# danieleschmidt/spin-torque-rl-gym

Measured on AMD Instinct MI355X. Metric: env_steps_per_sec, higher is better.
Workload: dtype f64

## Files before the change

### spin-torque-rl-gym_amd/csrc/stg_kernels.hpp

```cpp
#pragma once
#include "../../include/spintorque_hip.h"
#include "stg_launch_plan.hpp"
#include "stg_physics.hpp"

#include <hip/hip_runtime.h>

#include <type_traits>

using namespace stg;

struct alignas(16) EnvRec {
    double m[3];
    double tgt[3];
    double etot;
    uint32_t stepw;
    uint32_t rng;
};
static_assert(sizeof(EnvRec) == 64, "state record size");
constexpr uint32_t STG_DONE_BIT = 0x80000000u;

struct StateView {
    EnvRec* rec;
};

// ... 507 lines not shown
        } else {
            const int64_t p = IDS ? o : i;
            parse_action<AT>(act[p], act[N + p], a.c.max_current, a.c.max_duration, J, T);
        }
        if (MULTI) {
            const int c = (int)a.cls[i];
            row = s_tab + (c < a.ncls ? c : 0) * C_COUNT;
            k = load_llgs(row);
        }
        const RngKey rk{a.c.seed, (uint64_t)(a.env_id0 + i), rng};
        e_skip = a.c.skip_done && done;
        llgs_lane_begin<THERMAL, false, AXIS_Z>(L, out_m, m, J, T, k, row[C_BETA], row[C_BETAP], a.c.rtol, a.c.atol, a.c.max_step, rk,
                                                norec, noek, ns, !e_skip);
        has_env = true;
    };
    auto finish = [&]() {
        const SolveOut so = llgs_lane_finish<false>(L, out_m, norec, noek, ns);
        V3 m = L.m0, tgt = e_tgt;
        double etot = e_etot;
        int32_t step = e_step;
        uint32_t rng = e_rng;
        bool done = e_skip;
        env_step_tail(a, IDS ? o : i, 0, true, true, !e_skip, row, (uint64_t)(a.env_id0 + i), m, tgt, etot, step, rng, done, J, T, so, c_steps, c_sub, c_noop);
        store_state(a.s, i, m, tgt, etot, step, rng, done);
        has_env = false;
        L.active = false;
    };

    take(w * 64 + lane, true);
    const int64_t n_rest = nblk_q > nw ? nblk_q - nw : 0;
    static_assert(REFILL_STRIPES == 64, "one lane per stripe when a wavefront looks for a stripe that still has entries");
    int stripe = (int)(w % REFILL_STRIPES);
    bool queue_open = true;
    int64_t loc_q = 0, loc_end = 0;
    int loc_stripe = 0, full_streak = 0;
    bool more = n_rest > 0;
    const int check = a.refill_check > 0 ? a.refill_check : 1;
    for (;;) {
        LlgsMasks M = llgs_masks_open(L);
        for (int c = 0; c < check; ++c) {
            llgs_lane_gate<false>(L, M, (int32_t)a.c.max_attempts);
            if (M.active == 0ull) break;
            V3 z2{0.0, 0.0, 0.0}, z3{0.0, 0.0, 0.0};
            llgs_lane_attempt<THERMAL, false, AXIS_Z, false>(L, M, out_m, k, tb, a.c.rtol, a.c.atol, a.c.max_step, norec, noek, ns, z2, z3);
        }
        llgs_masks_close(L, M);
        const bool fin = has_env && !L.active;
        if (__ballot(fin) != 0ull || (more && __ballot(!has_env) != 0ull)) {
            if (fin) finish();
            const unsigned long long takers = __ballot(!has_env);
            if (more && takers != 0ull) {
                const int n_take = (int)__builtin_popcountll(takers), first = (int)__builtin_ctzll(takers);
                const int rank = (int)__builtin_popcountll(takers & ((1ull << lane) - 1ull));
                const int64_t avail = loc_end - loc_q;
                const int need_new = n_take > avail ? (int)(n_take - avail) : 0;
                int64_t new_q = 0;
                const int new_stripe = stripe;
                if (need_new > 0 && queue_open) {
                    const int reserve = (takers == ~0ull && full_streak >= 1) ? 4 * 64 : need_new;
                    unsigned long long base = 0;
                    if (lane == first) base = atomicAdd(a.refill_cursor + stripe * REFILL_CURSOR_STRIDE, (unsigned long long)reserve);
                    base = (unsigned long long)__shfl((long long)base, first);
                    new_q = (int64_t)base;
                    const int64_t stripe_end = ((n_rest - stripe + REFILL_STRIPES - 1) / REFILL_STRIPES) * 64;
                    int64_t new_end = new_q + reserve;
                    if (new_end >= stripe_end) {
                        new_end = stripe_end;
                        const int64_t end_l = ((n_rest - lane + REFILL_STRIPES - 1) / REFILL_STRIPES) * 64;
                        const unsigned long long cur_l = __hip_atomic_load(a.refill_cursor + lane * REFILL_CURSOR_STRIDE, __ATOMIC_RELAXED, __HIP_MEMORY_SCOPE_AGENT);
                        unsigned long long open_s = __ballot((int64_t)cur_l < end_l);
                        open_s &= ~(1ull << stripe);
                        if (open_s == 0ull) queue_open = false;
                        else {
                            const unsigned long long after = stripe == 63 ? 0ull : (open_s >> (stripe + 1)) << (stripe + 1);
                            stripe = (int)__builtin_ctzll(after != 0ull ? after : open_s);
                        }
                    }
                    const bool from_old = rank < avail;
                    const int64_t q = from_old ? loc_q + rank : new_q + (rank - avail);
                    const int st = from_old ? loc_stripe : new_stripe;
                    const int64_t r = (q >> 6) * REFILL_STRIPES + st;
                    take((nw + r) * 64 + (q & 63), !has_env && r < n_rest && (from_old || q < new_end));
                    loc_q = new_q + need_new < new_end ? new_q + need_new : new_end;
                    loc_end = new_end;
                    loc_stripe = new_stripe;
                } else {
                    const int64_t q = loc_q + rank;
                    const int64_t r = (q >> 6) * REFILL_STRIPES + loc_stripe;
                    take((nw + r) * 64 + (q & 63), !has_env && q < loc_end && r < n_rest);
                    loc_q = loc_q + n_take < loc_end ? loc_q + n_take : loc_end;
                }
                more = queue_open || loc_q < loc_end;
                full_streak = takers == ~0ull ? full_streak + 1 : 0;
            }
        }
        if (__ballot(has_env) == 0ull && !more) break;
    }
}

template <int SOLVER, bool THERMAL, int MULTI, bool AXIS_Z, bool DEVPHYS, typename AT, bool PC, int WGW, bool IDS>
#ifndef STG_STEP_ATTR
#define STG_STEP_ATTR
#endif
__global__ void __launch_bounds__(PC ? 2 * WGW * 64 : WGW * 64, (SOLVER != STG_SOLVER_RK45 && !THERMAL && !DEVPHYS && AXIS_Z && MULTI != 2 && !(MULTI && WGW == 1)) ? 4 : 1) STG_STEP_ATTR
stg_step_kernel(const StepArgs a) {
#pragma clang fp contract(off)
    static_assert(!PC || THERMAL, "wave specialisation only exists for the thermal kernels");
    extern __shared__ double s_tab[];
    constexpr bool FIELD = SOLVER == STG_SOLVER_RK45;
    using NT = typename std::conditional<FIELD, double, float>::type;
    constexpr bool BARRIER = SOLVER != STG_SOLVER_RK4;
    constexpr int DEPTH = BARRIER ? 2 : 4;
    constexpr int RING = DEPTH * (FIELD ? SHARED_CHUNK_RK45 : SHARED_CHUNK_FIXED) * 64;
    static_assert(!PC || WGW == 1, "the wave-specialised form is one integrating + one producing wavefront");
    __shared__ NT s_norm[PC ? RING : 1];
    __shared__ int s_hs[2], s_go[2 * WGW];
    __shared__ unsigned long long s_cnt[(PC ? 2 : 1) * WGW * 3];
    __shared__ uint32_t s_rng[PC ? WGW * 64 : 1];
    const int lane = (int)(threadIdx.x & 63u);
    const int wave = __builtin_amdgcn_readfirstlane((int)(threadIdx.x >> 6));
    bool paired = PC;
    int64_t hyb_slot = 0;
    if (PC && a.hybrid) hyb_slot = stg_hybrid_block(blockIdx.x, wave, (uint32_t)(a.hybrid - 1), (a.N + TILE_ENVS - 1) / TILE_ENVS, paired);
    const bool producer = PC && paired && wave >= WGW;
    const int cw = producer ? (2 * WGW - 1 - wave) : (wave < WGW ? wave : wave - WGW);
    record_placement(a.placement, wave, lane, producer);
    const int64_t lane_slot = ((PC && a.hybrid) ? hyb_slot
                                                : stg_slot_block<WGW>(blockIdx.x, (uint32_t)((a.N + WGW * 64 - 1) / (WGW * 64)), a.perm != nullptr, cw, PC,
                                                                      (uint32_t)a.snake_rounds) * 64) + lane;
    const bool in_list = lane_slot < a.N;
    const int64_t o = in_list ? (a.perm ? (int64_t)a.perm[lane_slot] : lane_slot) : 0;
    const uint32_t id = (IDS && in_list) ? a.ids[o] : 0u;
    const bool bad = IDS && in_list && (int64_t)id >= a.n_state;
    if (bad && !producer) write_bad_id(a, o);
    const bool live = in_list && !bad;
    const int64_t i = IDS ? (live ? (int64_t)id : 0) : o;
    constexpr int ENV_LAYOUT = SOLVER == STG_SOLVER_RK45 ? ENV_LAYOUT_LLGS : (DEVPHYS ? ENV_LAYOUT_DEV : ENV_LAYOUT_CORE);
    double own_row[MULTI == 2 ? C_COUNT : 1];
    const double* row;
    if constexpr (MULTI == 2) {
        stg_device_params p;
        load_env_params<ENV_LAYOUT>(a.ep, i, p);
        derive_row(p, a.ep.gamma, a.ep.temperature, own_row);
        row = own_row;
    } else {
        row = class_row<MULTI != 0>(a.ctab, a.cls, a.ncls, i, live, s_tab, a.ep, ENV_LAYOUT);
    }
    if (!PC && !live) return;
    if (PC && !paired && !live) return;
    const int64_t N = a.N;
    const uint64_t env_id = (uint64_t)(a.env_id0 + i);

    if (producer) {
        constexpr int n_first = SOLVER == STG_SOLVER_RK45 ? 6 : SHARED_CHUNK_FIXED;
        static_assert(3 * SHARED_SUBS3 == SHARED_CHUNK_FIXED, "chunk size of the 3-normal sub-steps");
        constexpr int n_chunk = SOLVER == STG_SOLVER_RK45 ? SHARED_CHUNK_RK45 : n_first;
        const double ghs = FIELD ? load_llgs(row).ghs : 0.0;
        for (int k = 0; k < a.K; ++k) {
            __syncthreads();
            const int p = (k & 1) * WGW;
            if (!any_flag<WGW>(lds_flag(s_go + p))) continue;
            const RngKey rk{a.c.seed, env_id, s_rng[cw * 64 + lane]};
            produce_normals<NT, FIELD, DEPTH, BARRIER>(s_norm, s_hs, lane, rk, n_first, n_chunk, ghs);
        }
        record_retired(a.placement, wave, lane, 0ull);
        return;
    }

    V3 m, tgt;
    double etot;
    int32_t step;
    uint32_t rng;
    bool done;
    load_state(a.s, i, m, tgt, etot, step, rng, done);
    const AT* act = (const AT*)a.actions;
    const Recorder norec{};
    unsigned long long c_steps = 0, c_sub = 0, c_noop = 0;

    for (int k = 0; k < a.K; ++k) {
        double J, T;
        if (k == 0 && a.perm) {
            typedef typename std::conditional<std::is_same<AT, double>::value, double2, float2>::type AT2;
            const AT2 aa = ((const AT2*)a.act_sorted)[live ? lane_slot : 0];
            parse_action<AT>(aa.x, aa.y, a.c.max_current, a.c.max_duration, J, T);
        } else {
            parse_action<AT>(act[((int64_t)k * 2 + 0) * N + o], act[((int64_t)k * 2 + 1) * N + o], a.c.max_current,
                             a.c.max_duration, J, T);
        }
        const bool last = (k == a.K - 1);
        const int64_t ko = a.out_every ? k : 0;
        const bool wr = (a.out_every || last) && live;
        const bool lane_solves = live && !(a.c.skip_done && done);
        const RngKey rk{a.c.seed, env_id, rng};
        SolveOut so{m, 0, 0, 0, false};
        if (PC && paired) {
            SharedNormalsT<NT, FIELD, DEPTH, BARRIER> shared{s_norm, s_hs, lane, 0, 0, 1};
            const int p = (k & 1) * WGW;
            s_rng[cw * 64 + lane] = rng;
            const bool mine = __ballot(lane_solves) != 0ull;
            s_go[p + cw] = mine ? 1 : 0;
            __syncthreads();
            if ((WGW == 1) ? mine : any_flag<WGW>(lds_flag(s_go + p))) {
                if (!BARRIER) s_hs[1] = 0;
                __syncthreads();
                so = run_solver<SOLVER, THERMAL, false, AXIS_Z, DEVPHYS>(m, J, T, row, a.c, rk, norec, shared, lane_solves);
            }
        }
        if (!(PC && paired) && lane_solves) {
            InlineNormals inl;
            so = run_solver<SOLVER, THERMAL, false, AXIS_Z, DEVPHYS>(m, J, T, row, a.c, rk, norec, inl, true);
        }
        env_step_tail(a, o, ko, wr, live, lane_solves, row, env_id, m, tgt, etot, step, rng, done, J, T, so, c_steps, c_sub, c_noop);
    }
    if (live) store_state(a.s, i, m, tgt, etot, step, rng, done);
    record_retired(a.placement, wave, lane, c_sub);
    const int ci = PC ? wave : cw;
    wave_add3(a.counters + (size_t)((blockIdx.x * (PC ? 2 : 1) * WGW + ci) % COUNTER_STRIPES) * COUNTER_STRIDE, s_cnt + ci * 3, c_steps, c_sub, c_noop);
}

template <bool THERMAL, bool MULTI, bool AXIS_Z, typename AT, int WGW, bool IDS>
__global__ void __launch_bounds__(WGW * 64) stg_step_refill_kernel(const StepArgs a) {
    extern __shared__ double s_tab[];
    __shared__ unsigned long long s_cnt[WGW * 3];
    const int lane = (int)(threadIdx.x & 63u);
    const int wave = __builtin_amdgcn_readfirstlane((int)(threadIdx.x >> 6));
    if (MULTI) {
        for (int j = threadIdx.x; j < a.ncls * C_COUNT; j += blockDim.x) s_tab[j] = a.ctab[j];
        __syncthreads();
    }
    const int64_t tiles = (a.N + TILE_ENVS - 1) / TILE_ENVS, nblk = tiles * TILE_WAVES, nw = a.refill_nw;
    const int64_t w = (int64_t)blockIdx.x * WGW + wave;
    record_placement(a.placement, wave, lane, false);
    if (w >= nw) return;
    unsigned long long c_steps = 0, c_sub = 0, c_noop = 0;
    refill_wave<THERMAL, MULTI, AXIS_Z, AT, IDS>(a, w, nw, 0, nblk, lane, s_tab, c_steps, c_sub, c_noop);
    refill_retire(a, w, nw, lane);
    record_retired(a.placement, wave, lane, c_sub);
    wave_add3(a.counters + (size_t)((blockIdx.x * WGW + wave) % COUNTER_STRIPES) * COUNTER_STRIDE, s_cnt + wave * 3, c_steps, c_sub, c_noop);
}

constexpr int64_t STG_WG4_MIN_ENVS = 65536;

template <class F>
static inline void with_flag(bool v, F&& f) {
    if (v) f(std::true_type{}); else f(std::false_type{});
}
template <class F>
static inline void with_multi(int multi, F&& f) {
    if (multi == 2) f(std::integral_constant<int, 2>{});
    else if (multi) f(std::integral_constant<int, 1>{});
    else f(std::integral_constant<int, 0>{});
}

template <int MULTI>
static size_t step_dyn_lds(const StepArgs& a) {
    return MULTI == 1 ? (size_t)a.ncls * C_COUNT * sizeof(double) : 0;
}

static inline unsigned step_grid(const StepArgs& a, int wgw) {
    const unsigned nwg = (unsigned)((a.N + wgw * 64 - 1) / (wgw * 64));
    if (!a.perm) return nwg;
    const unsigned tile_wgs = (unsigned)(TILE_WAVES / wgw);
    return ((nwg + tile_wgs - 1) / tile_wgs) * tile_wgs;
}

static int resident_workgroups_per_cu(const void* kernel, int block, size_t lds) {
    struct Key { const void* f; size_t lds; int v; };
    static thread_local Key cache[8] = {};
    static thread_local int used = 0;
    for (int j = 0; j < used; ++j) if (cache[j].f == kernel && cache[j].lds == lds) return cache[j].v;
    int nb = 0;
    if (hipOccupancyMaxActiveBlocksPerMultiprocessor(&nb, kernel, block, lds) != hipSuccess || nb < 1) nb = 2;
    if (used < 8) cache[used++] = Key{kernel, lds, nb};
    return nb;
}

static int32_t snake_rounds_of(const StepArgs& a, const void* kernel, int wgw, size_t lds) {
    if (!a.perm) return 0;
    const unsigned n_q = step_grid(a, wgw) / 8u;
    const int nb = resident_workgroups_per_cu(kernel, wgw * 64, lds);
    return (n_q > 32u && nb >= 2 && n_q <= 32u * (unsigned)nb + 16u) ? nb : 0;
}

template <int SOLVER, bool THERMAL, int MULTI, bool AXIS_Z, bool DEVPHYS, typename AT, bool PC, int WGW, bool IDS>
static void launch_step(const StepArgs& a, hipStream_t st) {
    if constexpr ((PC && (!THERMAL || DEVPHYS || WGW != 1)) || (DEVPHYS && SOLVER == STG_SOLVER_RK45)) return;
    else {
        const size_t lds = step_dyn_lds<MULTI>(a);
        StepArgs b = a;
        dim3 grid(step_grid(a, WGW));
        if constexpr (PC) {
            if (a.hybrid) grid = dim3(1024u);
            b.snake_rounds = (a.perm && step_grid(a, 1) / 8u <= 64u) ? 2 : 0;
        } else {
            b.snake_rounds = snake_rounds_of(a, (const void*)&stg_step_kernel<SOLVER, THERMAL, MULTI, AXIS_Z, DEVPHYS, AT, PC, WGW, IDS>, WGW, lds);
        }
        hipLaunchKernelGGL((stg_step_kernel<SOLVER, THERMAL, MULTI, AXIS_Z, DEVPHYS, AT, PC, WGW, IDS>), grid, dim3((PC ? 2 : 1) * WGW * 64), lds, st, b);
    }
}

template <int SOLVER, bool IDS>
static void dispatch_step(const StepArgs& a, bool thermal, int multi, bool axis_z, bool devphys, int act_f64, bool pc, hipStream_t st) {
    devphys = devphys && SOLVER != STG_SOLVER_RK45;
    pc = pc && thermal && !devphys;
    const bool wg4 = !pc && a.N >= STG_WG4_MIN_ENVS;
    with_flag(thermal, [&](auto THERMAL) { with_multi(multi, [&](auto MULTI) { with_flag(axis_z, [&](auto AXIS_Z) {
    with_flag(devphys, [&](auto DEVPHYS) { with_flag(act_f64 != 0, [&](auto F64) { with_flag(pc, [&](auto PC) { with_flag(wg4, [&](auto WG4) {
// ... 21 lines not shown
```

### spin-torque-rl-gym_amd/csrc/stg_physics.hpp

```cpp
#pragma once

#include <hip/hip_runtime.h>
#include <stdint.h>
#include <type_traits>

#include "stg_minstep.hpp"

namespace stg {

enum ClassConst : int {
    C_EX = 0, C_EY, C_EZ,
    C_HK,
    C_MS,
    C_ALPHA,
    C_GEFF,
    C_POL,
    C_MSV,
    C_HS_SIMPLE,
    C_RX, C_RY, C_RZ,
    C_DX, C_DY, C_DZ,
    C_HEX,
    C_BETA, C_BETAP,
    C_GAMMA,
    C_HS_LLGS,
// ... 86 lines not shown
__device__ __forceinline__ double vgpr_const(double c) {
    asm volatile("" : "+v"(c));
    return c;
}

__device__ __forceinline__ double fmax_abs(double a, double b) {
    double r;
    asm("v_max_f64 %0, |%1|, |%2|" : "=v"(r) : "v"(a), "v"(b));
    return r;
}

__device__ __forceinline__ void commit_step(unsigned long long mask, double& d0, double s0, double& d1, double s1, double& d2, double s2,
                                            double& d3, double s3, double& d4, double s4, double& d5, double s5, double& d6, double s6) {
    unsigned long long saved;
    asm("s_and_saveexec_b64 %[sv], %[m]\n\t"
        "v_mov_b64 %[d0], %[s0]\n\t"
        "v_mov_b64 %[d1], %[s1]\n\t"
        "v_mov_b64 %[d2], %[s2]\n\t"
        "v_mov_b64 %[d3], %[s3]\n\t"
        "v_mov_b64 %[d4], %[s4]\n\t"
        "v_mov_b64 %[d5], %[s5]\n\t"
        "v_mov_b64 %[d6], %[s6]\n\t"
        "s_mov_b64 exec, %[sv]"
        : [d0] "+v"(d0), [d1] "+v"(d1), [d2] "+v"(d2), [d3] "+v"(d3), [d4] "+v"(d4), [d5] "+v"(d5), [d6] "+v"(d6), [sv] "=&s"(saved)
        : [s0] "v"(s0), [s1] "v"(s1), [s2] "v"(s2), [s3] "v"(s3), [s4] "v"(s4), [s5] "v"(s5), [s6] "v"(s6), [m] "s"(mask)
        : "scc");
}

__device__ __forceinline__ double rcp_fast(double x) {
    const double y = __builtin_amdgcn_rcp(x);
    return __builtin_fma(y, __builtin_fma(-x, y, 1.0), y);
}

__device__ __forceinline__ double inv_tenth_root(double e2, double tenth = 0.1) {
    const double y = (double)__builtin_amdgcn_exp2f(-0.1f * __builtin_amdgcn_logf((float)e2));
    const double y2 = y * y, y4 = y2 * y2, y8 = y4 * y4;
    const double e = __builtin_fma(-e2, y8 * y2, 1.0);
    return __builtin_fma(y * e, __builtin_fma(0.055, e, tenth), y);
}

__device__ __forceinline__ double fifth_root(double x) {
    int e;
    const double mant = frexp(x, &e);
    const double t = -0.2 * ((double)e + (double)__builtin_amdgcn_logf((float)mant));
    const double ti = rint(t);
    double r = ldexp((double)__builtin_amdgcn_exp2f((float)(t - ti)), (int)ti);
    const double r2 = r * r, r4 = r2 * r2;
    const double err = __builtin_fma(-x, r4 * r, 1.0);
    r = __builtin_fma(r * err, __builtin_fma(0.12, err, 0.2), r);
    const double q2 = r * r;
    return x * (q2 * q2);
}

__device__ __forceinline__ V3 cross(const V3& a, const V3& b) {
#pragma clang fp contract(off)
    return V3{__builtin_fma(a.y, b.z, -(a.z * b.y)), __builtin_fma(a.z, b.x, -(a.x * b.z)), __builtin_fma(a.x, b.y, -(a.y * b.x))};
}
__device__ __forceinline__ double dot(const V3& a, const V3& b) {
#pragma clang fp contract(off)
    return __builtin_fma(a.z, b.z, __builtin_fma(a.y, b.y, a.x * b.x));
}
__device__ __forceinline__ V3 scale3(double c, const V3& z) {
#pragma clang fp contract(off)
    return V3{c * z.x, c * z.y, c * z.z};
}
__device__ __forceinline__ bool finite3(const V3& a) { return isfinite(a.x) && isfinite(a.y) && isfinite(a.z); }

__device__ __forceinline__ void philox4x32_10(uint32_t c0, uint32_t c1, uint32_t c2, uint32_t c3, uint32_t k0,
                                              uint32_t k1, uint32_t (&out)[4]) {
#pragma unroll
    for (int r = 0; r < 10; ++r) {
        const uint32_t hi0 = __umulhi(0xD2511F53u, c0), lo0 = 0xD2511F53u * c0;
        const uint32_t hi1 = __umulhi(0xCD9E8D57u, c2), lo1 = 0xCD9E8D57u * c2;
        const uint32_t n0 = hi1 ^ c1 ^ k0, n2 = hi0 ^ c3 ^ k1;
        c0 = n0; c1 = lo1; c2 = n2; c3 = lo0;
        k0 += 0x9E3779B9u; k1 += 0xBB67AE85u;
    }
    out[0] = c0; out[1] = c1; out[2] = c2; out[3] = c3;
}

struct NormalStream {
    uint32_t s0, s1, s2, s3;
    float carry;
    __device__ __forceinline__ void init(uint64_t seed, uint64_t env_id, uint32_t env_step, uint32_t tag) {
        uint32_t r[4];
        philox4x32_10((uint32_t)env_id, (uint32_t)(env_id >> 32), env_step, tag, (uint32_t)seed, (uint32_t)(seed >> 32), r);
        s0 = r[0]; s1 = r[1]; s2 = r[2]; s3 = r[3] | 1u;
        carry = 0.0f;
    }
    __device__ __forceinline__ uint32_t next() {
        const uint32_t result = s0 + s3;
        const uint32_t t = s1 << 9;
        s2 ^= s0; s3 ^= s1; s1 ^= s2; s0 ^= s3; s2 ^= t;
        s3 = (s3 << 11) | (s3 >> 21);
        return result;
    }
    __device__ __forceinline__ float uniform() {
        return __uint_as_float(__builtin_amdgcn_alignbit(0x7fu, next(), 9u)) - 0.99999994f;
    }
    typedef float f32x2 __attribute__((ext_vector_type(2)));
    __device__ __forceinline__ void pair(float& a, float& b) {
        float t, c, s_;
        pair_head(t, c, s_);
        finish_pair(t, c, s_, a, b);
    }
    __device__ __forceinline__ void pair_head(float& t, float& c, float& s_) {
        f32x2 u{__uint_as_float(__builtin_amdgcn_alignbit(0x7fu, next(), 9u)), __uint_as_float(__builtin_amdgcn_alignbit(0x7fu, next(), 9u))};
        u = u - f32x2{0.99999994f, 0.99999994f};
        t = -1.3862943611198906f * __builtin_amdgcn_logf(u.x);
        c = __builtin_amdgcn_cosf(u.y);
        s_ = __builtin_amdgcn_sinf(u.y);
    }
    static __device__ __forceinline__ void finish_pair(float t, float c, float s_, float& a, float& b) {
        const float r = __builtin_amdgcn_sqrtf(t);
        const f32x2 cs = f32x2{c, s_} * f32x2{r, r};
        a = cs.x;
        b = cs.y;
    }
    __device__ __forceinline__ V3 draw3_even() {
        float a, b, c, d;
        pair(a, b);
        pair(c, d);
        carry = d;
        return V3{(double)a, (double)b, (double)c};
    }
    __device__ __forceinline__ V3 draw3_odd() {
        float a, b;
        pair(a, b);
        return V3{(double)carry, (double)a, (double)b};
    }
};

struct RngKey {
    uint64_t seed, env_id;
    uint32_t env_step;
};

struct InlineNormals {
    static constexpr bool kShared = false, kScaled = false;
    NormalStream ns;
    __device__ __forceinline__ void begin(const RngKey& rk) { ns.init(rk.seed, rk.env_id, rk.env_step, 0u); }
    __device__ __forceinline__ V3 draw(bool even) { return even ? ns.draw3_even() : ns.draw3_odd(); }
    static constexpr bool broken = false;
    __device__ __forceinline__ void peek() {}
    __device__ __forceinline__ bool chunk_end(bool lane_continues) { return lane_continues; }
    __device__ __forceinline__ bool chunk_end_wave(bool mine) { return mine; }
    __device__ __forceinline__ int32_t chunk_end_go(int32_t go) { return go; }
};

constexpr int SHARED_SUBS_RK4 = 2;
constexpr int SHARED_SUBS3 = 4 * SHARED_SUBS_RK4;
constexpr int SHARED_CHUNK_FIXED = 12 * SHARED_SUBS_RK4;
constexpr int SHARED_CHUNK_RK45 = 18;
constexpr int PC_STOP = 1 << 30;
constexpr int PC_SPIN_CAP = 1 << 22;

typedef __attribute__((address_space(3))) int lds_int;
__device__ __forceinline__ volatile lds_int* lds_flag(const int* p) { return (volatile lds_int*)p; }

template <int WGW>
__device__ __forceinline__ bool any_flag(volatile lds_int* f) {
    int v = f[0];
#pragma unroll
    for (int j = 1; j < WGW; ++j) v |= f[j];
    return v != 0;
}
__device__ __forceinline__ int pc_load(const int* p) {
    return __builtin_amdgcn_readfirstlane(__hip_atomic_load(p, __ATOMIC_ACQUIRE, __HIP_MEMORY_SCOPE_WORKGROUP));
}
__device__ __forceinline__ void pc_store(int* p, int v) {
    __hip_atomic_store(p, v, __ATOMIC_RELEASE, __HIP_MEMORY_SCOPE_WORKGROUP);
}

template <typename T, bool SCALED, int DEPTH, bool BARRIER>
struct SharedNormalsT {
    static constexpr int CHUNK = SCALED ? SHARED_CHUNK_RK45 : SHARED_CHUNK_FIXED;
    static_assert(!BARRIER || DEPTH == 2, "the barrier form runs the producer exactly one chunk ahead");
    static constexpr bool kShared = true, kScaled = SCALED;
    const T* buf;
    int* hs;
    int lane, it, idx, seen;
    bool broken;
    static constexpr bool kToggle = BARRIER && SCALED;
    int slot_b, flag_b;
    __device__ __forceinline__ void begin(const RngKey&) {
        it = 0; idx = 0; seen = 1; broken = false;
        if (kToggle) {
            static_assert(((CHUNK * 64) & 63) == 0, "the slot bit and the lane bits are disjoint");
            slot_b = lane * (int)sizeof(T); flag_b = 0;
            asm volatile("" : "+v"(slot_b), "+v"(flag_b));
        }
    }
    __device__ __forceinline__ V3 draw(bool) {
        const T* b = kToggle ? (const T*)((const char*)buf + slot_b) + idx * 64 : buf + ((it & (DEPTH - 1)) * CHUNK + idx) * 64 + lane;
        idx += 3;
        return V3{(double)b[0], (double)b[64], (double)b[128]};
    }
    __device__ __forceinline__ void peek() {
        if (!BARRIER) seen = __hip_atomic_load(hs, __ATOMIC_RELAXED, __HIP_MEMORY_SCOPE_WORKGROUP);
    }
    __device__ __forceinline__ bool chunk_end(bool lane_continues) { return chunk_end_wave(__ballot(lane_continues) != 0ull); }
    __device__ __forceinline__ bool chunk_end_wave(bool mine) { return chunk_end_go(mine ? 1 : 0) != 0; }
    __device__ __forceinline__ int32_t chunk_end_go(int32_t go) {
        const bool mine = go != 0;
        if (BARRIER) {
            if (kToggle) {
                *(volatile lds_int*)((volatile __attribute__((address_space(3))) char*)lds_flag(hs) + flag_b) = go;
                flag_b ^= (int)sizeof(int); slot_b ^= CHUNK * 64 * (int)sizeof(T);
            } else {
                lds_flag(hs)[it & 1] = go;
            }
            __syncthreads();
            ++it;
            idx = 0;
            return go;
        }
        ++it;
        idx = 0;
        pc_store(hs + 1, it | (mine ? 0 : PC_STOP));
        int have = __builtin_amdgcn_readfirstlane(seen);
        if (__builtin_expect(mine && have <= it, 0)) {
            int spins = 0;
#pragma unroll 1
            do {
                if (spins) __builtin_amdgcn_s_sleep(1);
                have = pc_load(hs);
            } while (have <= it && ++spins <= PC_SPIN_CAP);
            broken = broken || have <= it;
        }
        seen = have;
        __builtin_amdgcn_fence(__ATOMIC_ACQUIRE, "workgroup");
        return (mine && !broken) ? 1 : 0;
    }
};

template <typename T, bool SCALED, int DEPTH, bool BARRIER>
__device__ __forceinline__ void produce_normals(T* buf, int* hs, int lane, const RngKey& rk, int n_first, int n_chunk, double c) {
    NormalStream ns;
    ns.init(rk.seed, rk.env_id, rk.env_step, 0u);
    bool even = true;
    auto fill = [&](int slot, int count) {
        T* b = buf + (slot * (SCALED ? SHARED_CHUNK_RK45 : SHARED_CHUNK_FIXED)) * 64 + lane;
        for (int j = 0; j < count; j += 3) {
            V3 z = even ? ns.draw3_even() : ns.draw3_odd();
            if (SCALED) z = scale3(c, z);
            even = !even;
            b[(j + 0) * 64] = (T)z.x; b[(j + 1) * 64] = (T)z.y; b[(j + 2) * 64] = (T)z.z;
        }
    };
    fill(0, n_first);
    if (!BARRIER) pc_store(hs, 1);
    __syncthreads();
    if (BARRIER) {
        for (int k = 1;; ++k) {
            fill(k & 1, n_chunk);
            __syncthreads();
            if (lds_flag(hs)[(k - 1) & 1] == 0) return;
        }
    }
    for (int k = 1;; ++k) {
        int v = pc_load(hs + 1);
#pragma unroll 1
        for (int spins = 0; (v & (PC_STOP - 1)) < k - DEPTH + 1 && !(v & PC_STOP); ++spins) {
            if (spins > PC_SPIN_CAP) return;
            __builtin_amdgcn_s_sleep(1);
            v = pc_load(hs + 1);
        }
        if (v & PC_STOP) return;
        fill(k & (DEPTH - 1), n_chunk);
        pc_store(hs, k + 1);
    }
}

struct SimpleK {
    V3 e;
    double ghk;
    double gdm;
    double alpha;
    double ghs;
};
__device__ __forceinline__ SimpleK make_simple(const V3& e, double hk, double ms, double alpha, double geff, double hs) {
#pragma clang fp contract(off)
    return SimpleK{e, -geff * hk, geff * ms, alpha, -geff * hs};
}
struct LlgsK {
    V3 r;
    V3 gd;
    double ghk, ghex;
    double alpha;
    double ghs;
    double gz;
    double agz;
};
__device__ __forceinline__ LlgsK make_llgs(const V3& r, const V3& d, double hk, double hex, double alpha, double gamma, double hs) {
#pragma clang fp contract(off)
    const double ng = -gamma;
    const double gz = ng * ((hk * r.z) * r.z + d.z);
    return LlgsK{r, V3{ng * d.x, ng * d.y, ng * d.z}, ng * hk, ng * hex, alpha, ng * hs, gz, alpha * gz};
}


template <bool THERMAL, bool AXIS_Z>
__device__ __forceinline__ V3 simple_rhs(const V3& m, const SimpleK& k, double ghk, double aJ, const V3& z) {
#pragma clang fp contract(off)
    if (AXIS_Z) {
        const double gz = (ghk + k.gdm) * m.z;
        V3 p;
        if (THERMAL) {
            const V3 g{k.ghs * z.x, k.ghs * z.y, __builtin_fma(k.ghs, z.z, gz)};
            p = cross(m, g);
        } else {
            p = V3{m.y * gz, -(m.x * gz), 0.0};
        }
        const double wx = __builtin_fma(k.alpha, p.x, aJ * m.y), wy = __builtin_fma(k.alpha, p.y, -(aJ * m.x));
        if (THERMAL) {
            const double wz = k.alpha * p.z;
            return V3{__builtin_fma(m.y, wz, __builtin_fma(-m.z, wy, p.x)), __builtin_fma(m.z, wx, __builtin_fma(-m.x, wz, p.y)),
                      __builtin_fma(m.x, wy, __builtin_fma(-m.y, wx, p.z))};
        }
        return V3{__builtin_fma(-m.z, wy, p.x), __builtin_fma(m.z, wx, p.y), __builtin_fma(m.x, wy, -(m.y * wx))};
    }
    const V3 t = cross(m, k.e);
    const double c = ghk * dot(m, k.e);
    const double d = k.gdm * m.z;
    V3 p;
    if (THERMAL) {
        const V3 g{__builtin_fma(k.ghs, z.x, c * k.e.x), __builtin_fma(k.ghs, z.y, c * k.e.y),
                   __builtin_fma(k.ghs, z.z, __builtin_fma(c, k.e.z, d))};
        p = cross(m, g);
    } else {
        p = V3{__builtin_fma(c, t.x, d * m.y), __builtin_fma(c, t.y, -(d * m.x)), c * t.z};
    }
    const V3 w{__builtin_fma(k.alpha, p.x, aJ * t.x), __builtin_fma(k.alpha, p.y, aJ * t.y),
               __builtin_fma(k.alpha, p.z, aJ * t.z)};
    return V3{__builtin_fma(m.y, w.z, __builtin_fma(-m.z, w.y, p.x)), __builtin_fma(m.z, w.x, __builtin_fma(-m.x, w.z, p.y)),
              __builtin_fma(m.x, w.y, __builtin_fma(-m.y, w.x, p.z))};
}

struct DevTorque {
    double sdl, sfl;
    V3 sigma;
    double ghk_pulse;
    bool any_sot;
};

__device__ __forceinline__ double vcma_keff(double volt, double ku, double xi, double td2, double vbd) {
    const double v = volt < -vbd ? -vbd : (volt > vbd ? vbd : volt);
    const double keff = ku + (-xi * fabs(v) / td2);
    return fmax(keff, -0.5 * ku);
}

template <bool THERMAL, bool AXIS_Z, bool DEVPHYS>
__device__ __forceinline__ V3 simple_stage(const V3& m, const SimpleK& k, double aJ, const V3& z, const DevTorque& dv,
                                           bool on) {
#pragma clang fp contract(off)
    if (!DEVPHYS) return simple_rhs<THERMAL, AXIS_Z>(m, k, k.ghk, aJ, z);
    V3 f = simple_rhs<THERMAL, AXIS_Z>(m, k, on ? dv.ghk_pulse : k.ghk, aJ, z);
    if (dv.any_sot) {
        const double a = on ? dv.sdl : 0.0, b = on ? dv.sfl : 0.0;
        const V3 sxm = cross(dv.sigma, m);
        f = V3{f.x + __builtin_fma(a, sxm.x, b * dv.sigma.x), f.y + __builtin_fma(a, sxm.y, b * dv.sigma.y),
               f.z + __builtin_fma(a, sxm.z, b * dv.sigma.z)};
    }
    return f;
}

__device__ __forceinline__ int simple_validate(V3& m, bool& zero_row) {
#pragma clang fp contract(off)
    zero_row = false;
    const double e = __builtin_fma(m.z, m.z, __builtin_fma(m.y, m.y, __builtin_fma(m.x, m.x, -1.0)));
    const bool near1 = fabs(e) < 0.0009765625;
    const double inv1 = __builtin_fma(e, __builtin_fma(e, __builtin_fma(e, __builtin_fma(e, 0.2734375, -0.3125), 0.375), -0.5), 1.0);
    if (__builtin_expect(__ballot(!near1) == 0ull, 1)) {
        m = V3{m.x * inv1, m.y * inv1, m.z * inv1};
        return 0;
    }
    const double s = dot(m, m);
    const double inv = near1 ? inv1 : rsqrt_fast(s);
    const bool ordinary = (s >= 1e-24) && (s <= 1.7976931348623157e308);
    if (__builtin_expect(__ballot(!ordinary) == 0ull, 1)) {
        m = V3{m.x * inv, m.y * inv, m.z * inv};
        return 0;
    }
    if (!finite3(m) || s < 1e-24) { m = V3{0.0, 0.0, 1.0}; return 1; }
    m = V3{m.x * inv, m.y * inv, m.z * inv};
    zero_row = isinf(s);
    return 0;
}

__device__ __forceinline__ bool validation_rejects(const V3& m) {
    return !finite3(m) || sqrt(dot(m, m)) < 1e-12;
}

struct SolveOut {
    V3 m;
    int32_t n;
    int32_t resets;
    int64_t work;
    bool ok;
};

struct Recorder {
    double* t;
// ... 149 lines not shown
         (c * k.r.z + k.gd.z * m.z) + k.ghex * m.z};
    if (THERMAL) g = V3{g.x + ht.x, g.y + ht.y, g.z + ht.z};
    const V3 U{g.x, g.y, g.z + bpJ};
    const V3 W{k.alpha * g.x, k.alpha * g.y, __builtin_fma(k.alpha, g.z, bJ)};
    const double s = dot(m, W);
    return V3{__builtin_fma(m.x, s, __builtin_fma(m.y, U.z, __builtin_fma(-m.z, U.y, -W.x))),
              __builtin_fma(m.y, s, __builtin_fma(m.z, U.x, __builtin_fma(-m.x, U.z, -W.y))),
              __builtin_fma(m.z, s, __builtin_fma(m.x, U.y, __builtin_fma(-m.y, U.x, -W.z)))};
}

struct LlgsEnergyK {
    double kuv, edemag;
    V3 r, nfac;
};
__device__ __forceinline__ double llgs_energy(const V3& m, const LlgsEnergyK& k) {
    const double ct = dot(m, k.r);
    return -k.kuv * (ct * ct) + k.edemag * (k.nfac.x * (m.x * m.x) + k.nfac.y * (m.y * m.y) + k.nfac.z * (m.z * m.z));
}

__device__ __forceinline__ double llgs_torque_norms(const V3& m, double bJ, double bpJ) {
#pragma clang fp contract(off)
    const V3 mxp{m.y, -m.x, 0.0};
    const V3 mm = cross(m, mxp);
    const V3 a{bJ * mm.x, bJ * mm.y, bJ * mm.z}, b{bpJ * mxp.x, bpJ * mxp.y, bpJ * mxp.z};
    return sqrt((a.x * a.x + a.y * a.y) + a.z * a.z) + sqrt((b.x * b.x + b.y * b.y) + b.z * b.z);
}

__device__ __forceinline__ double rms3(const V3& a) { return sqrt(dot(a, a)) / 1.7320508075688772; }

struct Dp5Tab {
    double A51, A52, A53, A54, A61, A62, A63, A64, A65, E1, E3, E4, E5, E6, E7;
    double B4, third, c09, tenth;
};
__device__ __forceinline__ Dp5Tab make_dp5_tab() {
    Dp5Tab t;
    t.A51 = vgpr_const(19372.0 / 6561); t.A52 = vgpr_const(-25360.0 / 2187); t.A53 = vgpr_const(64448.0 / 6561); t.A54 = vgpr_const(-212.0 / 729);
    t.A61 = vgpr_const(9017.0 / 3168); t.A62 = vgpr_const(-355.0 / 33); t.A63 = vgpr_const(46732.0 / 5247); t.A64 = vgpr_const(49.0 / 176);
    t.A65 = vgpr_const(-5103.0 / 18656);
    t.E1 = vgpr_const(-71.0 / 57600); t.E3 = vgpr_const(71.0 / 16695); t.E4 = vgpr_const(-71.0 / 1920); t.E5 = vgpr_const(17253.0 / 339200);
    t.E6 = vgpr_const(-22.0 / 525); t.E7 = vgpr_const(1.0 / 40);
    t.B4 = vgpr_const(125.0 / 192); t.third = vgpr_const(1.0 / 3.0); t.c09 = vgpr_const(0.9); t.tenth = vgpr_const(0.1);
    return t;
}

struct LlgsLane {
    V3 y, f;
    V3 m0;
    double t, T, h_abs;
    double h_floor;
    double bJ, bpJ;
    int32_t attempts;
    int32_t npts;
    bool idle;
    bool rejected, active;
};

typedef unsigned long long lanemask;
struct LlgsMasks {
    lanemask active, pacc, low;
};
__device__ __forceinline__ bool lane_in(lanemask m) { return __builtin_amdgcn_inverse_ballot_w64(m); }
__device__ __forceinline__ LlgsMasks llgs_masks_open(const LlgsLane& L) {
    return LlgsMasks{__ballot(L.active), __ballot(!L.rejected), __ballot(L.h_abs < L.h_floor)};
}
__device__ __forceinline__ void llgs_masks_close(LlgsLane& L, const LlgsMasks& M) {
    L.active = lane_in(M.active);
    L.rejected = !lane_in(M.pacc);
}

template <bool RECORD>
__device__ __forceinline__ void llgs_lane_emit(LlgsLane& L, V3& out_m, const Recorder& rec, const LlgsEnergyK& ek) {
    const double inv = rsqrt_fast(dot(L.y, L.y));
    out_m = V3{L.y.x * inv, L.y.y * inv, L.y.z * inv};
    if (RECORD) rec.put(L.npts, L.t, out_m, rec.e ? llgs_energy(out_m, ek) : 0.0, rec.tq ? llgs_torque_norms(out_m, L.bJ, L.bpJ) : 0.0);
    ++L.npts;
}

template <bool THERMAL, bool AXIS_Z, bool CHECKED = true>
__device__ __forceinline__ V3 llgs_fun(const LlgsLane& L, const LlgsK& k, const V3& y, const V3& ht, bool on) {
    return llgs_rhs<THERMAL, AXIS_Z, CHECKED>(y, k, on ? L.bJ : 0.0, on ? L.bpJ : 0.0, ht);
}
template <bool THERMAL, class NSRC>
__device__ __forceinline__ V3 llgs_draw(NSRC& ns, const LlgsK& k, bool even) {
    if (!THERMAL) return V3{0.0, 0.0, 0.0};
    return NSRC::kScaled ? ns.draw(even) : scale3(k.ghs, ns.draw(even));
}

template <bool THERMAL, bool RECORD, bool AXIS_Z, class NSRC>
__device__ __forceinline__ void llgs_lane_begin(LlgsLane& L, V3& out_m, const V3& m0, double J, double T, const LlgsK& k, double beta,
                                                double betap, double rtol, double atol, double max_step, const RngKey& rk,
                                                const Recorder& rec, const LlgsEnergyK& ek, NSRC& ns, bool enabled) {
    const bool useJ = !(fabs(J) < 1e-12);
    L.bJ = useJ ? beta * J : 0.0;
    L.bpJ = useJ ? betap * J : 0.0;
    L.m0 = m0;
    L.T = T;
    if (THERMAL) ns.begin(rk);
    const double n0 = rsqrt_fast(dot(m0, m0));
    L.y = V3{m0.x * n0, m0.y * n0, m0.z * n0};
    L.t = 0.0;
    L.npts = 0;
    if (RECORD) llgs_lane_emit<RECORD>(L, out_m, rec, ek); else ++L.npts;
    L.f = llgs_fun<THERMAL, AXIS_Z>(L, k, L.y, llgs_draw<THERMAL>(ns, k, true), true);
    double h_abs;
    {
        const V3& y = L.y;
        const V3& f = L.f;
        const V3 sc{atol + fabs(y.x) * rtol, atol + fabs(y.y) * rtol, atol + fabs(y.z) * rtol};
        const V3 isc{rcp_fast(sc.x), rcp_fast(sc.y), rcp_fast(sc.z)};
        const double d0 = rms3(V3{y.x * isc.x, y.y * isc.y, y.z * isc.z});
        const double d1 = rms3(V3{f.x * isc.x, f.y * isc.y, f.z * isc.z});
        double h0 = (d0 < 1e-5 || d1 < 1e-5) ? 1e-6 : (0.01 * d0) * rcp_fast(d1);
        h0 = fmin(h0, T);
        const V3 y1{y.x + h0 * f.x, y.y + h0 * f.y, y.z + h0 * f.z};
        const V3 f1 = llgs_fun<THERMAL, AXIS_Z>(L, k, y1, llgs_draw<THERMAL>(ns, k, false), true);
        const double d2 = rms3(V3{(f1.x - f.x) * isc.x, (f1.y - f.y) * isc.y, (f1.z - f.z) * isc.z}) * rcp_fast(h0);
        const double h1 = (d1 <= 1e-15 && d2 <= 1e-15) ? fmax(1e-6, h0 * 1e-3) : fifth_root(0.01 * rcp_fast(fmax(d1, d2)));
        h_abs = fmin(fmin(100.0 * h0, h1), fmin(T, max_step));
    }
    L.rejected = false;
    L.attempts = 0;
    const double min_step = min_step_at(L.t);
    L.h_abs = h_abs > max_step ? max_step : (h_abs < min_step ? min_step : h_abs);
    L.h_floor = isfinite(T) ? min_step_at(T) : __builtin_inf();
    L.active = enabled && (L.t != T);
    L.idle = !L.active;
}

template <bool UNIFORM_IT>
__device__ __forceinline__ void llgs_lane_gate(LlgsLane& L, LlgsMasks& M, int32_t max_attempts) {
    if (__builtin_expect((M.low & M.active) != 0ull, 0)) {
        const double min_step = min_step_at(L.t);
        if (lane_in(M.pacc)) L.h_abs = L.h_abs < min_step ? min_step : L.h_abs;
        M.active &= ~__ballot(L.h_abs < min_step);
    }
    if (!UNIFORM_IT) M.active &= ~__ballot(L.attempts >= max_attempts);
}

__device__ __forceinline__ int32_t attempt_loop_next(lanemask& active, lanemask not_arrived, int32_t& it, int32_t budget) {
    int32_t go;
    asm("s_add_i32 %[it], %[it], 1\n\t"
        "s_and_b64 %[act], %[act], %[na]\n\t"
        "s_cselect_b32 %[go], %[bud], 0\n\t"
        "s_cmp_lt_i32 %[it], %[go]\n\t"
        "s_cselect_b32 %[go], 1, 0"
        : [act] "+s"(active), [it] "+s"(it), [go] "=&s"(go)
        : [na] "s"(not_arrived), [bud] "s"(budget)
        : "scc");
    return go;
}

template <bool THERMAL, bool RECORD, bool AXIS_Z, bool UNIFORM_IT, class NSRC>
__device__ __forceinline__ void llgs_lane_attempt(LlgsLane& L, LlgsMasks& M, V3& out_m, const LlgsK& k, const Dp5Tab& tb, double rtol,
                                                  double atol, double max_step, const Recorder& rec, const LlgsEnergyK& ek, NSRC& ns, V3 z2, V3 z3) {
    constexpr double A21 = 1.0 / 5;
    constexpr double A31 = 3.0 / 40, A32 = 9.0 / 40;
    constexpr double A41 = 44.0 / 45, A42 = -56.0 / 15, A43 = 32.0 / 9;
    constexpr double B1 = 35.0 / 384, B3 = 500.0 / 1113, B5 = -2187.0 / 6784, B6 = 11.0 / 84;
    const double B4 = tb.B4;
    const double A51 = tb.A51, A52 = tb.A52, A53 = tb.A53, A54 = tb.A54, A61 = tb.A61, A62 = tb.A62, A63 = tb.A63, A64 = tb.A64, A65 = tb.A65;
    const double E1 = tb.E1, E3 = tb.E3, E4 = tb.E4, E5 = tb.E5, E6 = tb.E6, E7 = tb.E7;
    const double T = L.T;
    const bool active = lane_in(M.active);
    const V3 y = L.y;
    const double t = L.t;
    auto fun = [&](const V3& yy, const V3& ht, bool on) -> V3 { return llgs_fun<THERMAL, AXIS_Z, false>(L, k, yy, ht, on); };
    auto draw = [&](bool even) -> V3 { return llgs_draw<THERMAL>(ns, k, even); };
    L.attempts += active ? 1 : 0;
    const double t_new = fmin(add_x(t, L.h_abs), T);
    const double h = sub_x(t_new, t);
    const double h_try = fabs(h);
    const bool on_end = add_x(t, h) <= T;
    const V3 k1 = L.f;
    constexpr bool BATCH = THERMAL && NSRC::kShared;
    if (THERMAL && !NSRC::kShared) { z2 = draw(true); z3 = draw(false); }
    V3 y2{y.x + (k1.x * A21) * h, y.y + (k1.y * A21) * h, y.z + (k1.z * A21) * h};
    if (BATCH) batch_ready(y2.z, z2.x, z2.y, z2.z, z3.x, z3.y, z3.z);
    const V3 k2 = fun(y2, z2, true);
    V3 z4 = draw(true), z5{0.0, 0.0, 0.0};
    if (BATCH) { z5 = draw(false); __builtin_amdgcn_sched_barrier(0); }
    const V3 k3 = fun(V3{y.x + (k1.x * A31 + k2.x * A32) * h, y.y + (k1.y * A31 + k2.y * A32) * h,
                         y.z + (k1.z * A31 + k2.z * A32) * h}, z3, true);
    if (!BATCH) z5 = draw(false);
    V3 y4{y.x + (k1.x * A41 + k2.x * A42 + k3.x * A43) * h, y.y + (k1.y * A41 + k2.y * A42 + k3.y * A43) * h,
          y.z + (k1.z * A41 + k2.z * A42 + k3.z * A43) * h};
    if (BATCH) batch_ready(y4.z, z4.x, z4.y, z4.z, z5.x, z5.y, z5.z);
    const V3 k4 = fun(y4, z4, true);
    V3 z6 = draw(true), z7{0.0, 0.0, 0.0};
    if (BATCH) { z7 = draw(false); __builtin_amdgcn_sched_barrier(0); }
    const V3 k5 = fun(V3{y.x + (k1.x * A51 + k2.x * A52 + k3.x * A53 + k4.x * A54) * h,
                         y.y + (k1.y * A51 + k2.y * A52 + k3.y * A53 + k4.y * A54) * h,
                         y.z + (k1.z * A51 + k2.z * A52 + k3.z * A53 + k4.z * A54) * h}, z5, true);
    if (THERMAL) ns.peek();
    if (!BATCH) z7 = draw(false);
    V3 y6{y.x + (k1.x * A61 + k2.x * A62 + k3.x * A63 + k4.x * A64 + k5.x * A65) * h,
          y.y + (k1.y * A61 + k2.y * A62 + k3.y * A63 + k4.y * A64 + k5.y * A65) * h,
          y.z + (k1.z * A61 + k2.z * A62 + k3.z * A63 + k4.z * A64 + k5.z * A65) * h};
    if (BATCH) batch_ready(y6.z, z6.x, z6.y, z6.z, z7.x, z7.y, z7.z);
    const V3 k6 = fun(y6, z6, on_end);
    const V3 y_new{y.x + h * (k1.x * B1 + k3.x * B3 + k4.x * B4 + k5.x * B5 + k6.x * B6),
                   y.y + h * (k1.y * B1 + k3.y * B3 + k4.y * B4 + k5.y * B5 + k6.y * B6),
                   y.z + h * (k1.z * B1 + k3.z * B3 + k4.z * B4 + k5.z * B5 + k6.z * B6)};
    const V3 f_new = fun(y_new, z7, on_end);
    const V3 ev{(k1.x * E1 + k3.x * E3 + k4.x * E4 + k5.x * E5 + k6.x * E6 + f_new.x * E7) * h,
                (k1.y * E1 + k3.y * E3 + k4.y * E4 + k5.y * E5 + k6.y * E6 + f_new.y * E7) * h,
                (k1.z * E1 + k3.z * E3 + k4.z * E4 + k5.z * E5 + k6.z * E6 + f_new.z * E7) * h};
    const V3 sc{atol + fmax_abs(y.x, y_new.x) * rtol, atol + fmax_abs(y.y, y_new.y) * rtol, atol + fmax_abs(y.z, y_new.z) * rtol};
    const V3 q{ev.x * rcp_fast(sc.x), ev.y * rcp_fast(sc.y), ev.z * rcp_fast(sc.z)};
    const double err2 = dot(q, q) * tb.third;
    const double err = err2;
    const lanemask accm = M.active & __ballot(err < 1.0);
    const bool acc = lane_in(accm);
    const double r9 = tb.c09 * inv_tenth_root(err, tb.tenth);
    const double fa = fmin(lane_in(M.pacc) ? 10.0 : 1.0, r9);
    const double fr = fmax(0.2, r9);
    double h_next = fmin(h_try * (acc ? fa : fr), max_step);
    M.low = __ballot(h_next < L.h_floor);
    L.h_abs = h_next;
    commit_step(accm, L.t, t_new, L.y.x, y_new.x, L.y.y, y_new.y, L.y.z, y_new.z, L.f.x, f_new.x, L.f.y, f_new.y, L.f.z, f_new.z);
    if (RECORD) { if (acc) llgs_lane_emit<RECORD>(L, out_m, rec, ek); } else L.npts += acc ? 1 : 0;
    M.pacc = accm;
    if (!UNIFORM_IT) M.active &= __ballot(L.t != T);
}

template <bool RECORD, class NSRC>
__device__ __forceinline__ SolveOut llgs_lane_finish(LlgsLane& L, V3& out_m, const Recorder& rec, const LlgsEnergyK& ek, const NSRC& ns) {
    SolveOut o{L.m0, 0, 0, 0, false};
    if (!RECORD) { llgs_lane_emit<RECORD>(L, out_m, rec, ek); --L.npts; }
    o.m = out_m;
    o.n = L.npts - 1;
    o.work = L.attempts;
    const bool ok = L.idle || L.t == L.T;
    o.ok = ok && !ns.broken;
    if (!ok) o.m = L.m0;
    return o;
}

template <bool THERMAL, bool RECORD, bool AXIS_Z, class NSRC>
__device__ __forceinline__ SolveOut llgs_solve(const V3& m0, double J, double T, const LlgsK& k, double beta,
                                               double betap, double rtol, double atol, double max_step,
                                               int64_t max_attempts, const RngKey& rk, const Recorder& rec,
                                               const LlgsEnergyK& ek, NSRC& ns, bool enabled) {
    const Dp5Tab tb = make_dp5_tab();
    const V3 zero{0.0, 0.0, 0.0};
    LlgsLane L;
    V3 out_m = m0;
    llgs_lane_begin<THERMAL, RECORD, AXIS_Z>(L, out_m, m0, J, T, k, beta, betap, rtol, atol, max_step, rk, rec, ek, ns, enabled);
    LlgsMasks M = llgs_masks_open(L);
    atol = vgpr_const(atol);
    int32_t budget = (int32_t)max_attempts;
    asm volatile("" : "+s"(budget));
    int32_t it = 0;
    bool wave_go = M.active != 0ull;
    if (NSRC::kShared) wave_go = ns.chunk_end_wave(wave_go);
    if (wave_go)
    for (;;) {
      V3 z2 = zero, z3 = zero;
      if (THERMAL && NSRC::kShared) { z2 = llgs_draw<THERMAL>(ns, k, true); z3 = llgs_draw<THERMAL>(ns, k, false); }
      llgs_lane_gate<true>(L, M, budget);
      llgs_lane_attempt<THERMAL, RECORD, AXIS_Z, true>(L, M, out_m, k, tb, rtol, atol, max_step, rec, ek, ns, z2, z3);
      if (!ns.chunk_end_go(attempt_loop_next(M.active, __ballot(L.t != L.T), it, budget))) break;
    }
    llgs_masks_close(L, M);
    return llgs_lane_finish<RECORD>(L, out_m, rec, ek, ns);
}

__device__ __forceinline__ double resistance(const V3& m_in, int dev_type, double r_p, double r_ap, double tmr,
                                             const V3& ref, double r_series) {
#pragma clang fp contract(off)
    if (dev_type == 0) {
        const double inv = rsqrt_fast(dot(m_in, m_in));
        const V3 m{m_in.x * inv, m_in.y * inv, m_in.z * inv};
        const double r = r_p * (1.0 + tmr * (1.0 - dot(m, ref)) * 0.5);
        return fmax(r, r_p * 0.5);
    }
    double r = r_p + (r_ap - r_p) * (1.0 - dot(m_in, ref)) * 0.5;
    if (dev_type == 1) r = r + r_series;
    return fmax(r, 1.0);
}

template <typename AT>
__device__ __forceinline__ void parse_action(AT a0, AT a1, double max_current, double max_duration, double& J, double& T) {
    const AT cmax = (AT)1e8, dmin = (AT)1e-12, dmax = (AT)1e-6;
    if (!isnan(a0)) a0 = a0 < -cmax ? -cmax : (a0 > cmax ? cmax : a0);
    if (!isnan(a1)) a1 = a1 < dmin ? dmin : (a1 > dmax ? dmax : a1);
    if (isnan(a0) || isnan(a1) || isinf(a0) || isinf(a1)) { a0 = (AT)0; a1 = dmin; }
    const double j = (double)a0, t = (double)a1;
    J = j < -max_current ? -max_current : (j > max_current ? max_current : j);
    T = t < 1e-12 ? 1e-12 : (t > max_duration ? max_duration : t);
}

__device__ __forceinline__ float obs_cast(double v) {
    const float f = (float)v;
    return isnan(f) ? 0.0f : (isinf(f) ? (f > 0 ? 1e6f : -1e6f) : f);
}

}
```

Before: 44.21 million.

## Move RK45 chunk barrier mid-attempt and prefetch next attempt's first normals

```diff
diff --git a/spin-torque-rl-gym_amd/csrc/stg_kernels.hpp b/spin-torque-rl-gym_amd/csrc/stg_kernels.hpp
--- a/spin-torque-rl-gym_amd/csrc/stg_kernels.hpp
+++ b/spin-torque-rl-gym_amd/csrc/stg_kernels.hpp
@@ -683,7 +683,7 @@
     const uint64_t env_id = (uint64_t)(a.env_id0 + i);
 
     if (producer) {
-        constexpr int n_first = SOLVER == STG_SOLVER_RK45 ? 6 : SHARED_CHUNK_FIXED;
+        constexpr int n_first = SOLVER == STG_SOLVER_RK45 ? SHARED_FIRST_RK45 : SHARED_CHUNK_FIXED;
         static_assert(3 * SHARED_SUBS3 == SHARED_CHUNK_FIXED, "chunk size of the 3-normal sub-steps");
         constexpr int n_chunk = SOLVER == STG_SOLVER_RK45 ? SHARED_CHUNK_RK45 : n_first;
         const double ghs = FIELD ? load_llgs(row).ghs : 0.0;
diff --git a/spin-torque-rl-gym_amd/csrc/stg_physics.hpp b/spin-torque-rl-gym_amd/csrc/stg_physics.hpp
--- a/spin-torque-rl-gym_amd/csrc/stg_physics.hpp
+++ b/spin-torque-rl-gym_amd/csrc/stg_physics.hpp
@@ -262,6 +262,8 @@
 constexpr int SHARED_SUBS3 = 4 * SHARED_SUBS_RK4;
 constexpr int SHARED_CHUNK_FIXED = 12 * SHARED_SUBS_RK4;
 constexpr int SHARED_CHUNK_RK45 = 18;
+constexpr int SHARED_TAIL_RK45 = 6;
+constexpr int SHARED_FIRST_RK45 = 6 + SHARED_TAIL_RK45;
 constexpr int PC_STOP = 1 << 30;
 constexpr int PC_SPIN_CAP = 1 << 22;
 
@@ -306,6 +308,12 @@
         idx += 3;
         return V3{(double)b[0], (double)b[64], (double)b[128]};
     }
+    __device__ __forceinline__ void chunk_meet() {
+        __syncthreads();
+        slot_b ^= CHUNK * 64 * (int)sizeof(T);
+        idx = 0;
+    }
+    __device__ __forceinline__ void seek_tail() { idx = CHUNK - SHARED_TAIL_RK45; }
     __device__ __forceinline__ void peek() {
         if (!BARRIER) seen = __hip_atomic_load(hs, __ATOMIC_RELAXED, __HIP_MEMORY_SCOPE_WORKGROUP);
     }
@@ -313,13 +321,14 @@
     __device__ __forceinline__ bool chunk_end_wave(bool mine) { return chunk_end_go(mine ? 1 : 0) != 0; }
     __device__ __forceinline__ int32_t chunk_end_go(int32_t go) {
         const bool mine = go != 0;
+        if (kToggle) {
+            *(volatile lds_int*)((volatile __attribute__((address_space(3))) char*)lds_flag(hs) + flag_b) = go;
+            flag_b ^= (int)sizeof(int);
+            if (!mine) __syncthreads();
+            return go;
+        }
         if (BARRIER) {
-            if (kToggle) {
-                *(volatile lds_int*)((volatile __attribute__((address_space(3))) char*)lds_flag(hs) + flag_b) = go;
-                flag_b ^= (int)sizeof(int); slot_b ^= CHUNK * 64 * (int)sizeof(T);
-            } else {
-                lds_flag(hs)[it & 1] = go;
-            }
+            lds_flag(hs)[it & 1] = go;
             __syncthreads();
             ++it;
             idx = 0;
@@ -358,7 +367,15 @@
             b[(j + 0) * 64] = (T)z.x; b[(j + 1) * 64] = (T)z.y; b[(j + 2) * 64] = (T)z.z;
         }
     };
-    fill(0, n_first);
+    if constexpr (BARRIER && SCALED) {
+        fill(0, n_first - SHARED_TAIL_RK45);
+        T* ring = buf;
+        buf += (SHARED_CHUNK_RK45 - SHARED_TAIL_RK45) * 64;
+        fill(0, SHARED_TAIL_RK45);
+        buf = ring;
+    } else {
+        fill(0, n_first);
+    }
     if (!BARRIER) pc_store(hs, 1);
     __syncthreads();
     if (BARRIER) {
@@ -814,7 +831,7 @@
 
 template <bool THERMAL, bool RECORD, bool AXIS_Z, bool UNIFORM_IT, class NSRC>
 __device__ __forceinline__ void llgs_lane_attempt(LlgsLane& L, LlgsMasks& M, V3& out_m, const LlgsK& k, const Dp5Tab& tb, double rtol,
-                                                  double atol, double max_step, const Recorder& rec, const LlgsEnergyK& ek, NSRC& ns, V3 z2, V3 z3) {
+                                                  double atol, double max_step, const Recorder& rec, const LlgsEnergyK& ek, NSRC& ns, V3& z2, V3& z3) {
     constexpr double A21 = 1.0 / 5;
     constexpr double A31 = 3.0 / 40, A32 = 9.0 / 40;
     constexpr double A41 = 44.0 / 45, A42 = -56.0 / 15, A43 = 32.0 / 9;
@@ -839,6 +856,7 @@
     V3 y2{y.x + (k1.x * A21) * h, y.y + (k1.y * A21) * h, y.z + (k1.z * A21) * h};
     if (BATCH) batch_ready(y2.z, z2.x, z2.y, z2.z, z3.x, z3.y, z3.z);
     const V3 k2 = fun(y2, z2, true);
+    if constexpr (BATCH) ns.chunk_meet();
     V3 z4 = draw(true), z5{0.0, 0.0, 0.0};
     if (BATCH) { z5 = draw(false); __builtin_amdgcn_sched_barrier(0); }
     const V3 k3 = fun(V3{y.x + (k1.x * A31 + k2.x * A32) * h, y.y + (k1.y * A31 + k2.y * A32) * h,
@@ -864,6 +882,8 @@
                    y.y + h * (k1.y * B1 + k3.y * B3 + k4.y * B4 + k5.y * B5 + k6.y * B6),
                    y.z + h * (k1.z * B1 + k3.z * B3 + k4.z * B4 + k5.z * B5 + k6.z * B6)};
     const V3 f_new = fun(y_new, z7, on_end);
+    V3 z2n{0.0, 0.0, 0.0}, z3n{0.0, 0.0, 0.0};
+    if constexpr (BATCH) { z2n = draw(true); z3n = draw(false); __builtin_amdgcn_sched_barrier(0); }
     const V3 ev{(k1.x * E1 + k3.x * E3 + k4.x * E4 + k5.x * E5 + k6.x * E6 + f_new.x * E7) * h,
                 (k1.y * E1 + k3.y * E3 + k4.y * E4 + k5.y * E5 + k6.y * E6 + f_new.y * E7) * h,
                 (k1.z * E1 + k3.z * E3 + k4.z * E4 + k5.z * E5 + k6.z * E6 + f_new.z * E7) * h};
@@ -883,6 +903,7 @@
     if (RECORD) { if (acc) llgs_lane_emit<RECORD>(L, out_m, rec, ek); } else L.npts += acc ? 1 : 0;
     M.pacc = accm;
     if (!UNIFORM_IT) M.active &= __ballot(L.t != T);
+    if constexpr (BATCH) { z2 = z2n; z3 = z3n; }
 }
 
 template <bool RECORD, class NSRC>
@@ -915,10 +936,12 @@
     int32_t it = 0;
     bool wave_go = M.active != 0ull;
     if (NSRC::kShared) wave_go = ns.chunk_end_wave(wave_go);
+    V3 z2 = zero, z3 = zero;
+    if constexpr (THERMAL && NSRC::kShared) {
+        if (wave_go) { ns.seek_tail(); z2 = llgs_draw<THERMAL>(ns, k, true); z3 = llgs_draw<THERMAL>(ns, k, false); }
+    }
     if (wave_go)
     for (;;) {
-      V3 z2 = zero, z3 = zero;
-      if (THERMAL && NSRC::kShared) { z2 = llgs_draw<THERMAL>(ns, k, true); z3 = llgs_draw<THERMAL>(ns, k, false); }
       llgs_lane_gate<true>(L, M, budget);
       llgs_lane_attempt<THERMAL, RECORD, AXIS_Z, true>(L, M, out_m, k, tb, rtol, atol, max_step, rec, ek, ns, z2, z3);
       if (!ns.chunk_end_go(attempt_loop_next(M.active, __ballot(L.t != L.T), it, budget))) break;
```

Result: faster. 44.97 million, median of 6 (+1.7%).
